# Malfoy/Brisk

Hardware: AMD Instinct MI355X
Metric: distinct k-mers indexed/sec (k=63,m=21) (higher is better)
Workload: dtype u64; 1 GPU; 1x MI355X: 50M synthetic 150 bp reads per GPU, k=63 m=21 b=14, uint8 counts, 15x coverage; reads_per_gpu=50000000, total_reads=50000000, part_bits=24, genome_len=500000000, parallelism=single GPU

## Files before the change

### brisk_amd/csrc/brisk_scan.hip

```cpp
__global__ void __launch_bounds__(256) k_pack_ascii(const uint8_t* __restrict__ bases, u64 n_bases, u32* __restrict__ packed, u64 n_words) {
    const u64 w = (u64)blockIdx.x * blockDim.x + threadIdx.x;
    if (w >= n_words) return;
    const u64 base = w * 16;
    u32 v = 0;
    if (base + 16 <= n_bases && ((uintptr_t)(bases + base) & 15) == 0) {
        const uint4 q = *reinterpret_cast<const uint4*>(bases + base);
        const u32 ws[4] = {q.x, q.y, q.z, q.w};
#pragma unroll
        for (int i = 0; i < 4; i++) {
#pragma unroll
            for (int j = 0; j < 4; j++) v = (v << 2) | ((ws[i] >> (8 * j + 1)) & 3u);
        }
    } else {
        for (int i = 0; i < 16; i++) {
            const u64 p = base + i;
            const u32 c = p < n_bases ? ((bases[p] >> 1) & 3u) : 0u;
            v = (v << 2) | c;
        }
    }
    packed[w] = v;
}

__device__ __forceinline__ u64 sm_mix(u64 z) {
    z = (z ^ (z >> 30)) * 0xBF58476D1CE4E5B9ull;
// ... 117 lines not shown
                s.rev = c != fwd;
            } else if (d == s.pos) {
                if (canon < 0) {
                    const u64 hi = K > 32 ? load_nts(packed, q, K - 32) : 0;
                    canon = canonized_as_executed(mk128(low, hi), K) ? 1 : 0;
                }
                if (!canon) {
                    s.pos = d;
                    s.mini = c;
                    s.rev = false;
                }
            }
        }
    }
    return s;
}

template <bool CLS>
__device__ __forceinline__ u32 superkmer_pieces(const BriskParams& P, u32 n, u32 idx_end) {
    return (CLS ? P.cls_bits : 0u) ? cls_of(P, idx_end) - cls_of(P, idx_end - (n - 1)) + 1 : 1u;
}

__device__ __forceinline__ W4 x_shr(W4 a, u32 s) { return w4_shr(a, s); }
__device__ __forceinline__ W4 x_shl(W4 a, u32 s) { return w4_shl(a, s); }
__device__ __forceinline__ W4 x_and(W4 a, W4 b) { return w4_and(a, b); }
__device__ __forceinline__ W4 x_andn(W4 a, W4 b) { return w4_andn(a, b); }
__device__ __forceinline__ W4 x_or(W4 a, W4 b) { return w4_or(a, b); }
__device__ __forceinline__ W4 x_xor(W4 a, W4 b) { return W4{a.w0 ^ b.w0, a.w1 ^ b.w1, a.w2 ^ b.w2, a.w3 ^ b.w3}; }
__device__ __forceinline__ W4 x_rc(W4 a, u32 len) { return w4_rc(a, len); }
__device__ __forceinline__ u64 x_w0(W4 a) { return a.w0; }
__device__ __forceinline__ u64 x_word(W4 a, u32 i) { return i == 0 ? a.w0 : i == 1 ? a.w1 : i == 2 ? a.w2 : a.w3; }
__device__ __forceinline__ u128x x_shr(u128x a, u32 s) { return shr128(a, s); }
__device__ __forceinline__ u128x x_shl(u128x a, u32 s) { return shl128(a, s); }
__device__ __forceinline__ u128x x_and(u128x a, u128x b) { return and128(a, b); }
__device__ __forceinline__ u128x x_andn(u128x a, u128x b) { return andn128(a, b); }
__device__ __forceinline__ u128x x_or(u128x a, u128x b) { return or128(a, b); }
__device__ __forceinline__ u128x x_xor(u128x a, u128x b) { return u128x{a.lo ^ b.lo, a.hi ^ b.hi}; }
__device__ __forceinline__ u128x x_rc(u128x a, u32 len) {
    const u64 c = 0xaaaaaaaaaaaaaaaaull;
    return shr128(u128x{rev_nts64(a.hi ^ c), rev_nts64(a.lo ^ c)}, 128 - 2 * len);
}
__device__ __forceinline__ u64 x_w0(u128x a) { return a.lo; }
__device__ __forceinline__ u64 x_word(u128x a, u32 i) { return i == 0 ? a.lo : i == 1 ? a.hi : 0ull; }
template <class T> __device__ __forceinline__ T x_mask(u32 bits);
template <> __device__ __forceinline__ W4 x_mask<W4>(u32 bits) { return w4_mask(bits); }
template <> __device__ __forceinline__ u128x x_mask<u128x>(u32 bits) { return mask128(bits); }
template <class T> __device__ __forceinline__ T x_from64(u64 v);
template <> __device__ __forceinline__ W4 x_from64<W4>(u64 v) { return W4{v, 0, 0, 0}; }
template <> __device__ __forceinline__ u128x x_from64<u128x>(u64 v) { return u128x{v, 0}; }
template <class T> __device__ __forceinline__ T x_load(const u32* __restrict__ packed, u64 q, u32 len);
template <> __device__ __forceinline__ W4 x_load<W4>(const u32* __restrict__ packed, u64 q, u32 len) { return load_span(packed, q, len); }
template <> __device__ __forceinline__ u128x x_load<u128x>(const u32* __restrict__ packed, u64 q, u32 len) {
    const u32 c = len >= 32 ? 32 : len;
    u128x r{load_nts(packed, q + len - c, c), 0};
    if (len > 32) r.hi = load_nts(packed, q, len - 32);
    return r;
}

template <bool CLS, class T, bool POS = false>
__device__ __forceinline__ void emit_record_wide(const BriskParams& P, const u32* __restrict__ packed, u64 q0, u32 p0, u32 n, bool rev,
                                                 u32 idx_end, const ScanOut& out, u32 tag, u64 ret, unsigned long long slot) {
    const u32 L = P.k + n - 1;
    T S = x_load<T>(packed, q0 + p0, L);
    if (rev) S = x_rc(S, L);
    const u64 mm = x_w0(x_shr(S, 2 * idx_end)) & P.m_mask;
    const u64 h = mix2m(mm, P.m_mask);
    const u32 rbase = routing_base(P, h);
    S = x_xor(S, x_shl(x_from64<T>(mm ^ h), 2 * idx_end));
    const u32 cut = idx_end + P.suff_reduc;
    const T lowm = x_mask<T>(2 * cut);
    const T C = x_or(x_andn(x_shr(S, 2 * P.b), lowm), x_and(S, lowm));
    const u32 idx_first = idx_end - (n - 1);

    for (u32 j0 = 0; j0 < n;) {
        u32 j1 = n, bucket = rbase;
        if ((CLS ? P.cls_bits : 0u)) {
            const u32 c = cls_of(P, idx_first + j0);
            if (c + 1 < (1u << (CLS ? P.cls_bits : 0u))) j1 = min(n, (c + 1) * P.cls_width - idx_first);
            bucket = (rbase << (CLS ? P.cls_bits : 0u)) | c;
        }
        const u32 np = j1 - j0;
        T Cp = C;
        if (np != n) Cp = x_and(x_shr(C, 2 * (n - j1)), x_mask<T>(2 * (P.kb + np - 1)));
        u64* r;
        if (out.bins) {
            const u32 part = bucket >> P.shift;
#ifdef SCAN_ATTR_NOATOMIC
            const u32 rank = (part * 7u + (threadIdx.x & 63)) % out.bin_cap;
#else
            const u32 rank = (u32)atomicAdd(&out.hist[part], 1ull | ((unsigned long long)np << 32));
#endif
            if (rank < out.bin_cap) {
                r = out.bins + ((u64)part * out.bin_cap + rank) * P.stride;
                if (POS) {
                    const u64 ti = (u64)part * out.bin_cap + rank;
                    out.tag[ti] = (u32)ti;
                    out.ret[ti] = ret;
                } else if (out.tag) out.tag[(u64)part * out.bin_cap + rank] = tag;
            } else {
                const u32 reg = part & (OVF_REGIONS - 1);
                const u32 at = atomicAdd(&out.ovf_cnt[reg], 1u);
                if (at >= out.ovf_region_cap) {
                    *out.overflow = 1;
                    return;
                }
                const u64 o = (u64)reg * out.ovf_region_cap + at;
                r = out.ovf + o * P.stride;
                if (POS) {
                    const u64 ti = ((u64)out.bin_cap << P.part_bits) + o;
                    out.tag[ti] = (u32)ti;
                    out.ret[ti] = ret;
                } else if (out.tag) out.tag[((u64)out.bin_cap << P.part_bits) + o] = tag;
            }
        } else {
            r = out.rec + slot * P.stride;
        }
#ifdef SCAN_ATTR_NOSTORE
        if ((x_word(Cp, 0) ^ x_word(Cp, 1)) == 0x123456789abcdefull)
#endif
        {
            r[0] = x_word(Cp, 0);
            if (P.nw > 1) r[1] = x_word(Cp, 1);
            if (P.nw > 2) r[2] = x_word(Cp, 2);
            if (P.nw > 3) r[3] = x_word(Cp, 3);
            r[P.nw] = rec_header(bucket, np, idx_first + j0 + P.suff_reduc);
        }
        if (!out.bins) {
            if (out.tag) out.tag[slot] = tag;
            if (out.ret) out.ret[slot] = ret;
            if (out.hist) atomicAdd(&out.hist[bucket >> P.shift], 1ull | ((unsigned long long)np << 32));
        }
        slot++;
        j0 = j1;
    }
}
#ifndef EMIT_SMALL
#define EMIT_SMALL 1
#endif
template <bool CLS, bool POS = false>
__device__ void emit_record_at(const BriskParams& P, const u32* __restrict__ packed, u64 q0, u32 p0, u32 n, bool rev,
                               u32 idx_end, const ScanOut& out, u32 tag, u64 ret, unsigned long long slot) {
    if (!out.bins && slot + superkmer_pieces<CLS>(P, n, idx_end) > out.cap) {
        *out.overflow = 1;
        return;
    }
    if (EMIT_SMALL && 2 * P.k - P.m <= 64) emit_record_wide<CLS, u128x, POS>(P, packed, q0, p0, n, rev, idx_end, out, tag, ret, slot);
    else emit_record_wide<CLS, W4, POS>(P, packed, q0, p0, n, rev, idx_end, out, tag, ret, slot);
}
__device__ void emit_record(const BriskParams& P, const u32* __restrict__ packed, u64 q0, u32 p0, u32 n, bool rev,
                            u32 idx_end, const ScanOut& out, u32 tag, u64 ret = 0) {
    emit_record_at<true>(P, packed, q0, p0, n, rev, idx_end, out, tag, ret, atomicAdd(out.n_rec, (unsigned long long)superkmer_pieces<true>(P, n, idx_end)));
}

__global__ void __launch_bounds__(SCAN_BLOCK) k_scan(BriskParams P, const u32* __restrict__ packed, const u64* __restrict__ starts,
                                                     u64 n_reads, const double* __restrict__ g_coef, ScanOut out, int query_mode) {
    __shared__ double s_coef[128];
    for (u32 i = threadIdx.x; i < 4 * P.m; i += blockDim.x) s_coef[i] = g_coef[i];
    __syncthreads();
    const u64 r = (u64)blockIdx.x * blockDim.x + threadIdx.x;
    if (r >= n_reads) return;
    const u64 q0 = starts[r];
    const u64 len = starts[r + 1] - q0;
    const u32 k = P.k, m = P.m, w = P.w;
    if (len < k) return;
    const u64 M = P.m_mask;

    u64 cf = 0, cr = 0;
    for (u32 i = 0; i < m; i++) {
        const u32 c = nt_at(packed, q0 + k - m - 1 + i);
        cf = ((cf << 2) + c) & (M >> 2);
        cr = (cr >> 2) + ((u64)(c ^ 2u) << (2 * m - 2));
    }
    MiniState st = rescan_minimizer(packed, q0, k - 1, m, M, s_coef);
    u64 mini_hash = order_key(st.mini, m, M, s_coef);
    u32 mini_pos = st.pos;
    bool reversed = st.rev;
    u64 mini = st.mini;

    const u32 nk = (u32)(len - k + 1);
    u32 n = 0, p0 = 0, first_idx = 0, last_idx = 0, n_emitted = 0;
    for (u32 p = 0; p < nk; p++) {
        const u32 c = nt_at(packed, q0 + k - 1 + p);
        cf = ((cf << 2) + c) & M;
        cr = (cr >> 2) + ((u64)(c ^ 2u) << (2 * m - 2));
        mini_pos++;
        const u64 cand = cf < cr ? cf : cr;
        const u64 h = order_key(cand, m, M, s_coef);
        bool closed = false;
        const bool old_rev = reversed;
        u64 ret = 0;
        if (mini_pos > w) {
            closed = true;
            ret = mini;
            st = rescan_minimizer(packed, q0 + p, k, m, M, s_coef);
            mini = st.mini;
            mini_pos = st.pos;
            reversed = st.rev;
            mini_hash = order_key(mini, m, M, s_coef);
        } else if (h < mini_hash) {
            closed = true;
            ret = mini;
            mini_hash = h;
            mini_pos = 0;
            mini = cand;
            reversed = cand == cr;
        }
        const u32 idx = reversed ? w - mini_pos : mini_pos;
        if (closed && p > 0) {
            if (query_mode && n_emitted > 0 && ret == 0) return;
            emit_record(P, packed, q0, p0, n, old_rev, old_rev ? first_idx : last_idx, out, out.ret ? p0 : (u32)r, ret);
            n_emitted++;
            n = 0;
        }
        if (n == 0) {
            p0 = p;
            first_idx = idx;
        }
        last_idx = idx;
        n++;
    }
    if (n > 0) {
        if (query_mode && n_emitted > 0 && mini == 0) return;
        emit_record(P, packed, q0, p0, n, reversed, reversed ? first_idx : last_idx, out, out.ret ? p0 : (u32)r, mini);
    }
}

__device__ __forceinline__ unsigned long long lanes_below(u32 lane) { return (1ull << lane) - 1; }

#ifndef CLS_W
#define CLS_W 5
#endif
__host__ __device__ constexpr u32 cls_nch(u32 m) { return (m + CLS_W - 1) / CLS_W; }
__host__ __device__ constexpr u32 cls_width(u32 m, u32 c) {
    return m / cls_nch(m) + (c < m % cls_nch(m) ? 1u : 0u);
}
__host__ __device__ constexpr u32 cls_off(u32 m, u32 c) {
    u32 o = 0;
    for (u32 j = 0; j < c; j++) o += cls_width(m, j);
    return o;
}
__host__ __device__ constexpr u32 cls_base(u32 m, u32 c) {
    u32 b = 0;
    for (u32 j = 0; j < c; j++) b += 1u << (2 * cls_width(m, j));
    return b;
}
#define CLS_MAX_CHUNKS 8

struct ScanCfg {
    u32 nlow;
    u32 nlow1;
    u32 nch;
    u32 qcap;
    u32 n_tab;
    u32 chunk[CLS_MAX_CHUNKS];
};

#define CLS_HI 21
#define CLS_LO 12
#define CLS_BIAS 0x80000000u
__host__ __device__ constexpr u32 scan_fixed_tabs(int MM) { return MM > 0 ? 128 + cls_base((u32)MM, cls_nch((u32)MM)) : 0u; }
template <int NCH, int MM>
__device__ __forceinline__ u64 cls_sums(u64 x, const ScanCfg& cfg, const u64* tabs) {
    u64 acc;
    if (MM > 0) {
        constexpr u32 mm = MM > 0 ? (u32)MM : 1u;
        const char* tb = (const char*)tabs;
        const u32 xl = (u32)x, xh = (u32)(x >> 32);
        acc = *(const u64*)(tb + ((xl << 3) & (((1u << (2 * cls_width(mm, 0))) - 1) << 3)));
#pragma unroll
        for (u32 c = 1; c < cls_nch(mm); c++) {
            const u32 lo = 2 * cls_off(mm, c), wd = 2 * cls_width(mm, c), mk = ((1u << wd) - 1) << 3;
            u32 bo;
            if (lo + wd <= 32) bo = xl >> (lo - 3);
            else if (lo >= 35) bo = xh >> (lo - 35);
            else if (lo >= 32) bo = xh << (35 - lo);
            else bo = (u32)(x >> (lo - 3));
            acc += *(const u64*)(tb + 8 * cls_base(mm, c) + (bo & mk));
        }
    } else if (NCH > 0) {
        acc = tabs[(u32)x & ((1u << ((cfg.chunk[0] >> 6) & 15)) - 1)];
#pragma unroll
        for (int c = 1; c < NCH; c++) {
            const u32 d = cfg.chunk[c];
            acc += tabs[(d >> 10) + ((u32)(x >> (d & 63)) & ((1u << ((d >> 6) & 15)) - 1))];
        }
    } else {
        acc = tabs[(u32)x & ((1u << ((cfg.chunk[0] >> 6) & 15)) - 1)];
        for (u32 c = 1; c < cfg.nch; c++) {
            const u32 d = cfg.chunk[c];
            acc += tabs[(d >> 10) + ((u32)(x >> (d & 63)) & ((1u << ((d >> 6) & 15)) - 1))];
        }
    }
    return acc;
}
template <int NCH, int MM>
__device__ __forceinline__ u32 decy_class_guarded(u64 x, const ScanCfg& cfg, const u64* tabs, bool& guard) {
    const u64 acc = cls_sums<NCH, MM>(x, cfg, tabs);
    const u32 a = (u32)acc, b = (u32)(acc >> 32);
    const u32 da = ((a > CLS_BIAS ? a : CLS_BIAS) - (a < CLS_BIAS ? a : CLS_BIAS)) + (0u - (CLS_LO + 1));
    const u32 db = ((b > CLS_BIAS ? b : CLS_BIAS) - (b < CLS_BIAS ? b : CLS_BIAS)) + (0u - (CLS_LO + 1));
    guard = guard | ((da < db ? da : db) <= (u32)(CLS_HI - CLS_LO - 2));
    const bool c0 = a >= CLS_BIAS + CLS_HI && b <= CLS_BIAS + CLS_LO, c1 = a <= CLS_BIAS - CLS_HI && b >= CLS_BIAS - CLS_LO;
#ifdef CLS_FORCE_GUARD
    guard = true;
#endif
    return c0 ? 0u : c1 ? 1u : 2u;
// ... 169 lines not shown
    const u32 slot = tags[i];
    if (i < n_spec_end && (status[slot] & CHUNK_RERUN)) return;
    const u64 r = ret[i], q = r & 0x7fffffffffffffffull;
    const VRead v = vreads[slot];
    if ((r >> 63) && q > starts[v.read]) atomicMin(&brk[v.first], (unsigned long long)q);
}
__global__ void __launch_bounds__(256) k_query_filter(BriskParams P, const u64* __restrict__ rec, const u64* __restrict__ ret, const u32* __restrict__ tags, u64 first,
                                                      u64 n_spec_end, u64 n_rec, const VRead* __restrict__ vreads, const u32* __restrict__ status,
                                                      const unsigned long long* __restrict__ brk, u64* __restrict__ out, u32* __restrict__ tag_out,
                                                      unsigned long long* __restrict__ n_out) {
    const u64 i = first + (u64)blockIdx.x * blockDim.x + threadIdx.x;
    if (i >= n_rec) return;
    const u32 slot = tags[i];
    if (i < n_spec_end && (status[slot] & CHUNK_RERUN)) return;
    const VRead v = vreads[slot];
    if ((ret[i] & 0x7fffffffffffffffull) >= brk[v.first]) return;
    const unsigned long long o = atomicAdd(n_out, 1ull);
    for (u32 j = 0; j < P.stride; j++) out[o * P.stride + j] = rec[i * P.stride + j];
    tag_out[o] = v.read;
}
__global__ void __launch_bounds__(256) k_filter_records(BriskParams P, const u64* __restrict__ rec, const u32* __restrict__ tags, u64 first, u64 n_rec,
                                                        const u32* __restrict__ status, u64* __restrict__ out, unsigned long long* __restrict__ n_out) {
    const u64 i = first + (u64)blockIdx.x * blockDim.x + threadIdx.x;
    if (i >= n_rec) return;
    if (status[tags[i]] & CHUNK_RERUN) return;
    const unsigned long long slot = atomicAdd(n_out, 1ull);
    for (u32 j = 0; j < P.stride; j++) out[slot * P.stride + j] = rec[i * P.stride + j];
}

#define SLOT_ITEMS 16
__device__ __forceinline__ u64 read_slots(const u64* __restrict__ starts, u64 r, u32 k) {
    const u64 len = starts[r + 1] - starts[r];
    return len >= k ? len - k + 1 : 0;
}
__global__ void __launch_bounds__(256) k_slot_block(const u64* __restrict__ starts, u64 n_reads, u32 k, u64* __restrict__ block_sums) {
    __shared__ u64 s[4];
    const u64 base = (u64)blockIdx.x * 256 * SLOT_ITEMS;
    u64 acc = 0;
    for (int i = 0; i < SLOT_ITEMS; i++) {
        const u64 r = base + (u64)i * 256 + threadIdx.x;
        if (r < n_reads) acc += read_slots(starts, r, k);
    }
    for (int o = 32; o > 0; o >>= 1) acc += __shfl_down(acc, o, 64);
    if ((threadIdx.x & 63) == 0) s[threadIdx.x >> 6] = acc;
    __syncthreads();
    if (threadIdx.x == 0) block_sums[blockIdx.x] = s[0] + s[1] + s[2] + s[3];
}
__global__ void __launch_bounds__(1024) k_slot_top(u64* __restrict__ block_sums, u32 nb) {
    __shared__ u64 s_wave[16];
    __shared__ u64 s_carry;
    if (threadIdx.x == 0) s_carry = 0;
    __syncthreads();
    for (u32 base = 0; base < nb; base += 1024) {
        const u32 i = base + threadIdx.x;
        const u64 v = i < nb ? block_sums[i] : 0;
        u64 x = v;
        for (int o = 1; o < 64; o <<= 1) {
            const u64 y = __shfl_up(x, o, 64);
            if ((int)(threadIdx.x & 63) >= o) x += y;
        }
        if ((threadIdx.x & 63) == 63) s_wave[threadIdx.x >> 6] = x;
        __syncthreads();
        u64 woff = 0;
        for (u32 j = 0; j < (threadIdx.x >> 6); j++) woff += s_wave[j];
        const u64 carry = s_carry;
        if (i < nb) block_sums[i] = carry + woff + x - v;
        __syncthreads();
        if (threadIdx.x == 1023) s_carry = carry + woff + x;
        __syncthreads();
    }
    if (threadIdx.x == 0) block_sums[nb] = s_carry;
}
__global__ void __launch_bounds__(256) k_slot_apply(const u64* __restrict__ starts, u64 n_reads, u32 k, const u64* __restrict__ block_sums,
                                                    u64* __restrict__ slot_base) {
    __shared__ u64 s_wave[4];
    const u64 base = (u64)blockIdx.x * 256 * SLOT_ITEMS + (u64)threadIdx.x * SLOT_ITEMS;
    u64 tsum = 0;
    for (int i = 0; i < SLOT_ITEMS; i++)
        if (base + i < n_reads) tsum += read_slots(starts, base + i, k);
    u64 x = tsum;
    for (int o = 1; o < 64; o <<= 1) {
        const u64 y = __shfl_up(x, o, 64);
        if ((int)(threadIdx.x & 63) >= o) x += y;
    }
    if ((threadIdx.x & 63) == 63) s_wave[threadIdx.x >> 6] = x;
    __syncthreads();
    u64 woff = 0;
    for (u32 j = 0; j < (threadIdx.x >> 6); j++) woff += s_wave[j];
    u64 run = block_sums[blockIdx.x] + woff + x - tsum;
    for (int i = 0; i < SLOT_ITEMS; i++) {
        const u64 r = base + i;
        if (r >= n_reads) break;
        slot_base[r] = run - starts[r];
        run += read_slots(starts, r, k);
    }
}
__global__ void __launch_bounds__(256) k_chunk_slot_base(const VRead* __restrict__ vreads, u32 n_chunks, const u64* __restrict__ slot_base, u64* __restrict__ out) {
    const u32 i = blockIdx.x * blockDim.x + threadIdx.x;
    if (i < n_chunks) out[i] = slot_base[vreads[i].read];
}
__global__ void __launch_bounds__(256) k_pos_filter(BriskParams P, const u64* __restrict__ rec, const u64* __restrict__ anchor, const u32* __restrict__ tags, u64 first,
                                                    u64 n_spec_end, u64 n_rec, const u32* __restrict__ status, u64* __restrict__ out, u64* __restrict__ anchor_out,
                                                    unsigned long long* __restrict__ n_out) {
    const u64 i = first + (u64)blockIdx.x * blockDim.x + threadIdx.x;
    if (i >= n_rec) return;
    if (i < n_spec_end && (status[tags[i]] & CHUNK_RERUN)) return;
    const unsigned long long o = atomicAdd(n_out, 1ull);
    for (u32 j = 0; j < P.stride; j++) out[o * P.stride + j] = rec[i * P.stride + j];
    anchor_out[o] = anchor[i];
}

__device__ __forceinline__ void resolve_ties(u32 first, u32 last, bool rev_first, bool rev_last, u32 Km, bool canon_if_needed_known, bool canon,
                                             u32* pos, bool* rev, bool* need_canon) {
    *need_canon = false;
    *pos = first;
    *rev = rev_first;
    if (last != first) {
        const u32 dT = Km - last;
        if (dT < first) {
            *pos = dT;
            *rev = rev_last;
        } else if (dT == first) {
            if (!canon_if_needed_known) *need_canon = true;
            else if (!canon) *rev = false;
        }
    }
}

__device__ __forceinline__ u64 pos_anchor(const BriskParams& P, u64 slot_base, u64 q, u32 n, bool rev, u32 idx_end) {
    const u64 g = rev ? q + idx_end : q + P.w - idx_end + n - 1;
    return (slot_base + g) | (rev ? 1ull << 63 : 0ull);
}

template <bool CLS, bool POS = false>
__device__ __forceinline__ void emit_queued(const BriskParams& P, const u32* __restrict__ packed, const ScanOut& out, u64 ent, const u64* s_q0, const u32* s_tag,
                                            unsigned long long slot, const u64* slot_base) {
    const u32 mi = (u32)(ent >> 32), src = (mi >> 18) & 63u;
    const u64 q_start = s_q0[src] + (u32)ent;
    const u64 ret = POS ? pos_anchor(P, slot_base[s_tag[src]], q_start, mi & 0xff, (mi >> 16) & 1, (mi >> 8) & 0xff) : q_start | ((u64)((mi >> 17) & 1) << 63);
    emit_record_at<CLS, POS>(P, packed, q_start, 0, mi & 0xff, (mi >> 16) & 1, (mi >> 8) & 0xff, out, s_tag[src], ret, slot);
}

template <bool CLS>
__device__ __forceinline__ u32 queue_records(const BriskParams& P, const u64* q_ent, u32 qcount) {
    if (!(CLS ? P.cls_bits : 0u)) return qcount;
    u32 mine = 0;
    for (u32 e = threadIdx.x & 63; e < qcount; e += 64) {
        const u32 mi = (u32)(q_ent[e] >> 32);
        mine += superkmer_pieces<CLS>(P, mi & 0xff, (mi >> 8) & 0xff);
    }
    for (int o = 32; o > 0; o >>= 1) mine += __shfl_xor(mine, o, 64);
    return mine;
}
template <bool CLS, bool POS = false>
__device__ __forceinline__ void emit_queue(const BriskParams& P, const u32* __restrict__ packed, const ScanOut& out, const u64* q_ent, const u64* s_q0, const u32* s_tag,
                                           u32 qcount, unsigned long long base, const u64* slot_base = nullptr) {
    const u32 lane = threadIdx.x & 63;
    if (!(CLS ? P.cls_bits : 0u)) {
        for (u32 e = lane; e < qcount; e += 64) emit_queued<CLS, POS>(P, packed, out, q_ent[e], s_q0, s_tag, base + e, slot_base);
        return;
    }
    for (u32 e0 = 0; e0 < qcount; e0 += 64) {
        const u32 e = e0 + lane;
        u64 ent = 0;
        u32 np = 0;
        if (e < qcount) {
            ent = q_ent[e];
            const u32 mi = (u32)(ent >> 32);
            np = superkmer_pieces<CLS>(P, mi & 0xff, (mi >> 8) & 0xff);
        }
        u32 incl = np;
        for (int o = 1; o < 64; o <<= 1) {
            const u32 y = __shfl_up(incl, o, 64);
            if ((int)lane >= o) incl += y;
        }
        if (e < qcount) emit_queued<CLS, POS>(P, packed, out, ent, s_q0, s_tag, base + incl - np, slot_base);
        base += (u32)__shfl(incl, 63, 64);
    }
}

template <bool CLS, bool POS = false>
__device__ __forceinline__ void scan_final_flush(const BriskParams& P, const u32* __restrict__ packed, const ScanOut& out, const u64* q_ent, const u64* s_q0,
                                                 const u32* s_tag, u32 qcount, u32* s_wcnt, unsigned long long* s_wbase, const u64* slot_base = nullptr) {
    const u32 lane = threadIdx.x & 63, wid = threadIdx.x >> 6, nw = blockDim.x >> 6;
    const u32 n_mine = queue_records<CLS>(P, q_ent, qcount);
    if (out.bins) {
        if (lane == 0 && n_mine) atomicAdd(out.n_rec, (unsigned long long)n_mine);
        emit_queue<CLS, POS>(P, packed, out, q_ent, s_q0, s_tag, qcount, 0, slot_base);
        return;
    }
    if (lane == 0) s_wcnt[wid] = n_mine;
    __syncthreads();
    if (threadIdx.x == 0) {
        u32 total = 0;
        for (u32 i = 0; i < nw; i++) total += s_wcnt[i];
        *s_wbase = total ? atomicAdd(out.n_rec, (unsigned long long)total) : 0ull;
    }
    __syncthreads();
    unsigned long long base = *s_wbase;
    for (u32 i = 0; i < wid; i++) base += s_wcnt[i];
    emit_queue<CLS, POS>(P, packed, out, q_ent, s_q0, s_tag, qcount, base, slot_base);
}

__device__ __forceinline__ u32 row_min_u32(u32 x) {
#define ROW_MIN_STEP(CTRL)                                                                      \
    {                                                                                           \
        const u32 y_ = (u32)__builtin_amdgcn_update_dpp((int)x, (int)x, CTRL, 0xf, 0xf, false); \
        x = y_ < x ? y_ : x;                                                                    \
    }
    ROW_MIN_STEP(0x128)
    ROW_MIN_STEP(0x124)
    ROW_MIN_STEP(0x122)
    ROW_MIN_STEP(0x121)
#undef ROW_MIN_STEP
    return x;
}

struct MinQueue {
    u64 k0, k1, k2;
    u32 meta;
};
#define MQ_EMPTY (~0ull)
#define MQ_TRUNC (1u << 30)
__device__ __forceinline__ void mq_reset(MinQueue& q, u64 key, u32 birth, bool rv, bool trunc) {
    q.k0 = key;
    q.k1 = q.k2 = MQ_EMPTY;
    q.meta = (birth & 0xffu) | (rv ? 1u << 24 : 0u) | (trunc ? MQ_TRUNC : 0u);
}
__device__ __forceinline__ void mq_push(MinQueue& q, u64 h, u32 step, bool rv) {
    const bool l0 = q.k0 < h, l1 = q.k1 < h, l2 = q.k2 < h;
    const bool e0 = q.k0 == h, e1 = q.k1 == h, e2 = q.k2 == h;
    const u32 cnt = (q.k0 != MQ_EMPTY ? 1u : 0u) + (q.k1 != MQ_EMPTY ? 1u : 0u) + (q.k2 != MQ_EMPTY ? 1u : 0u);
    const u32 keep = (l0 ? 1u : 0u) + (l1 ? 1u : 0u) + (l2 ? 1u : 0u);
    if (e0 | e1 | e2) {
        const u32 j = e0 ? 0u : e1 ? 1u : 2u;
        if (j < 1) q.k1 = MQ_EMPTY;
        if (j < 2) q.k2 = MQ_EMPTY;
        q.meta |= (1u << (27 + j)) | MQ_TRUNC;
        return;
    }
    const bool store = keep < 3 && (!(q.meta & MQ_TRUNC) || keep < cnt);
    if (!store) {
        q.meta |= MQ_TRUNC;
        return;
    }
    const u32 sh = 8 * keep;
    q.meta = (q.meta & ~((0xffu << sh) | (1u << (24 + keep)) | (1u << (27 + keep)) | MQ_TRUNC)) | ((step & 0xffu) << sh) | (rv ? 1u << (24 + keep) : 0u);
    if (keep == 0) q.k0 = h;
    if (keep <= 1) q.k1 = keep == 1 ? h : MQ_EMPTY;
    if (keep <= 2) q.k2 = keep == 2 ? h : MQ_EMPTY;
}
__device__ __forceinline__ void mq_pop_front(MinQueue& q) {
    q.k0 = q.k1;
    q.k1 = q.k2;
    q.k2 = MQ_EMPTY;
    q.meta = ((q.meta >> 8) & 0xffffu) | (((q.meta >> 25) & 3u) << 24) | (((q.meta >> 28) & 3u) << 27) | (q.meta & MQ_TRUNC);
}

#ifdef BRISK_PHASE_PROF
__device__ unsigned long long g_scan_cnt[8];
#define SCNT(i, v) scan_cnt[i] += (v);
#else
#define SCNT(i, v)
#endif

#ifndef SCAN_WAVES_PER_EU
#define SCAN_WAVES_PER_EU 6
#endif
__host__ __device__ constexpr int scan_waves_per_eu(int KK, int MM) { return KK && MM >= 12 ? SCAN_WAVES_PER_EU : 4; }
template <int NCH, int MODE, int KK, int MM>
__global__ void __launch_bounds__(1024) __attribute__((amdgpu_waves_per_eu(scan_waves_per_eu(KK, MM), 8))) k_scan2(BriskParams P, ScanCfg cfg, const u32* __restrict__ packed, const u64* __restrict__ starts,
                                                u64 n_reads, const double* __restrict__ g_tabs, ScanOut out, ChunkCtl cc) {
    constexpr bool VR = MODE == 2 || MODE == 4, query_mode = MODE == 1, POS = MODE >= 3;
    constexpr bool CLS = MM < 12;
    extern __shared__ double smem_dyn[];
    const u32 tid = threadIdx.x, lane = tid & 63, wid = tid >> 6;
    const u32 n_tab = MM ? 128 + cls_base(MM ? MM : 1, cls_nch(MM ? MM : 1)) : cfg.n_tab;
    double* smem_d = smem_dyn;
    double* smem_q = smem_dyn + n_tab;
    if constexpr (scan_fixed_tabs(MM) > 0) {
        __shared__ double s_fix[scan_fixed_tabs(MM)];
        smem_d = s_fix;
        smem_q = smem_dyn;
    }
    const double* s_coef = smem_d;
    const u64* s_tabs = (const u64*)(smem_d + 128);
    for (u32 i = tid; i < n_tab; i += blockDim.x) smem_d[i] = g_tabs[i];
    unsigned long long* s_wbase = (unsigned long long*)smem_q;
    u32* s_wcnt = (u32*)(s_wbase + 1);
    u64* q_ent = (u64*)(smem_q + 9) + (size_t)wid * (cfg.qcap + 96);
    u64* s_q0 = q_ent + cfg.qcap;
    u32* s_tag = (u32*)(s_q0 + 64);

    if (KK) {
        P.k = KK;
        P.w = KK - MM;
    }
    if (MM) {
        P.m = MM;
        P.m_mask = (1ull << (2 * MM)) - 1;
    }
    const u32 k = KK ? (u32)KK : P.k, m = MM ? (u32)MM : P.m, w = k - m;
    const u64 M = MM ? ((1ull << (2 * MM)) - 1) : P.m_mask;
    const u32 ksh = 2 * m > 30 ? 2 * m - 30 : 0;
    const u32 nlow = k < 32 ? k : 32, nlow1 = k - 1 < 32 ? k - 1 : 32;
    const u64 r = (u64)blockIdx.x * blockDim.x + tid;
    u64 q0 = 0, len = 0;
    u32 emit_from = 0, emit_until = 0xffffffffu, tagval = (u32)r, vslot = 0;
    bool seq_first = true, seq_last = true, seeded = false;
    if (r < n_reads) {
        if (VR) {
            const VRead v = cc.vreads[r];
            q0 = v.q0;
            len = v.len;
            emit_from = v.emit_from;
            emit_until = v.emit_until;
            tagval = vslot = v.slot;
            seq_first = v.flags & 1u;
            seq_last = v.flags & 2u;
            seeded = v.flags & 4u;
        } else {
            q0 = starts[r];
            len = starts[r + 1] - q0;
            if (cc.long_limit && len >= k && len - k + 1 > cc.long_limit) len = 0;
        }
    }
    s_q0[lane] = q0;
    s_tag[lane] = tagval;
    __syncthreads();
    const bool live = len >= k;
    u32 nk = live ? (u32)(len - k + 1) : 0;
    u32 max_nk = nk;
    for (int o = 32; o > 0; o >>= 1) {
        const u32 y = __shfl_xor(max_nk, o, 64);
        max_nk = y > max_nk ? y : max_nk;
    }
    if (max_nk == 0) {
        scan_final_flush<CLS, POS>(P, packed, out, q_ent, s_q0, s_tag, 0, s_wcnt, s_wbase, cc.slot_base);
        return;
    }
    const u64 KEY0 = order_key_fast<NCH, MM>(0, m, M, cfg, s_tabs, s_coef);
    const u64 KEY0s = read_lane_u64(KEY0, 0);

    u64 cr = 0, low64 = 0;
    if (live) low64 = load_nts(packed, q0 + (k - 1) - nlow1, nlow1);
    cr = rc64(low64 & M, m);

    u64 mini_hash;
    u32 mini_pos;
    bool reversed;
#ifndef SCAN_MINQUEUE
#define SCAN_MINQUEUE 1
#endif
#ifndef PROLOGUE_UNROLL
#define PROLOGUE_UNROLL 2
#endif
#define BRISK_PRAGMA_(x) _Pragma(#x)
#define BRISK_PRAGMA(x) BRISK_PRAGMA_(x)
    const bool mq_on = SCAN_MINQUEUE && (KK ? (KK <= 32) : (k <= 32));
    MinQueue mq{MQ_EMPTY, MQ_EMPTY, MQ_EMPTY, 0u};
    {
        const u32 Km = k - 1 - m;
        const u32 nwin = Km + 1 < nlow1 ? Km + 1 : nlow1;
        struct WinMin {
            u64 best;
            u32 first, last, flags;
        };
        auto pass = [&](auto exact_tag) -> WinMin {
            constexpr bool EXACT = decltype(exact_tag)::value;
            u64 best = ~0ull;
            u32 first = 0, last = 0, rf = 0, rl = 0;
            bool guard = false;
            u64 fw = low64 & M, rw = cr, above = low64 >> (2 * m);
            if (mq_on) mq = MinQueue{MQ_EMPTY, MQ_EMPTY, MQ_EMPTY, 0u};
#ifdef SCAN_ATTR_NOPROLOGUE
            for (u32 ii = 0; ii < 1; ii++) {
#else
            BRISK_PRAGMA(unroll PROLOGUE_UNROLL)
            for (u32 ii = 0; ii < nwin; ii++) {
#endif
                const u32 i = mq_on ? Km - ii : ii;
                u64 fwd, rcv;
                if (mq_on) {
                    fwd = (low64 >> (2 * i)) & M;
                    rcv = rc64(fwd, m);
                } else {
                    fwd = fw;
                    rcv = rw;
                    const u32 t = (u32)above & 3u;
                    above >>= 2;
                    fw = (fw >> 2) | ((u64)t << (2 * m - 2));
                    rw = ((rw << 2) & M) | (t ^ 2u);
                }
                const bool rv = rcv < fwd;
                const u64 x = rv ? rcv : fwd;
                u64 key;
                if (EXACT) key = order_key(x, m, M, s_coef);
                else {
#ifdef SCAN_ATTR_NOCLASS
                    key = order_key_fast<NCH, MM>(x, m, M, cfg, s_tabs, s_coef);
#else
                    key = ((u64)decy_class_guarded<NCH, MM>(x, cfg, s_tabs, guard) << 62) + mix2m(x, M);
#endif
                }
                const bool lt = key < best, eq = key == best;
                best = lt ? key : best;
                if (mq_on) {
                    first = lt || eq ? i : first;
                    rf = lt || eq ? (u32)rv : rf;
                    last = lt ? i : last;
                    rl = lt ? (u32)rv : rl;
                } else {
                    first = lt ? i : first;
                    rf = lt ? (u32)rv : rf;
                    last = lt || eq ? i : last;
                    rl = lt || eq ? (u32)rv : rl;
                }
                if (mq_on) mq_push(mq, key, 0u - 1u - i, rv);
            }
            return WinMin{best, first, last, rf | (rl << 1) | (guard ? 4u : 0u)};
        };
#ifdef SCAN_ATTR_PROLOGUE_TWICE
        if (__ballot(pass(std::false_type{}).flags & 4u) == 0x123456789ull) return;
        __builtin_amdgcn_s_barrier();
#endif
        WinMin wm = pass(std::false_type{});
        if (__ballot(wm.flags & 4u)) wm = pass(std::true_type{});
        u64 best = wm.best;
        u32 first = wm.first, last = wm.last;
        bool rf = wm.flags & 1u, rl = wm.flags & 2u;
        if (Km >= nwin) {
            if (KEY0 < best) {
                best = KEY0;
                first = nwin;
                last = Km;
                rf = rl = false;
            } else if (KEY0 == best) {
                last = Km;
                rl = false;
            }
        }
        u32 pos;
        bool rev, need_canon;
        resolve_ties(first, last, rf, rl, Km, false, false, &pos, &rev, &need_canon);
        if (need_canon && live) {
            const u64 hi = k - 1 > 32 ? load_nts(packed, q0, k - 1 - 32) : 0;
            if (!canonized_as_executed(mk128(low64, hi), k - 1)) rev = false;
        }
        mini_hash = best;
        mini_pos = pos;
        reversed = rev;
        if (mq_on && last != first) mq_reset(mq, best, 0u - 1u - pos, rev, true);
    }
    if (seeded) {
        const ChunkState st = cc.truth[vslot];
        mini_hash = st.hash;
        mini_pos = st.pos_rev & 0x7fffffffu;
        reversed = st.pos_rev >> 31;
        if (mq_on) mq_reset(mq, mini_hash, 0u - 1u - mini_pos, reversed, true);
    }
    bool foreign = seeded;

    u32 qcount = 0;
    u32 p0 = 0, n_emitted = 0;
    bool dead = false;
    u64 buf = 0;
    const u32 Km = k - m;
    const u32 lane_bits = lane << 18;
#ifdef BRISK_PHASE_PROF
    unsigned long long scan_cnt[8] = {0, 0, 0, 0, 0, 0, 0, 0};
#endif
    for (u32 p = 0; p < max_nk; p++) {
        SCNT(0, 1)
        const bool act = p < nk && !dead;
        if (VR && live) {
            if (p == emit_from && !seq_first && !seeded) cc.spec[vslot] = ChunkState{mini_hash, mini_pos | ((reversed ? 1u : 0u) << 31), 1u};
            if (p == emit_until) cc.truth[vslot + 1] = ChunkState{mini_hash, mini_pos | ((reversed ? 1u : 0u) << 31), 1u};
        }
        if ((p & 31) == 0 && p < nk) {
            const u32 left = (u32)(len - (k - 1 + p));
            const u32 cnt = left < 32 ? left : 32;
            buf = load_nts(packed, q0 + k - 1 + p, cnt) << (64 - 2 * cnt);
        }
        const u32 c = (u32)(buf >> 62);
        buf <<= 2;
        cr = (cr >> 2) + ((u64)(c ^ 2u) << (2 * m - 2));
        low64 = (low64 << 2) | c;
        const u64 cf = low64 & M;
        const bool revf = cr < cf;
        const u64 h = order_key_fast<NCH, MM>(revf ? cr : cf, m, M, cfg, s_tabs, s_coef);
        mini_pos += act ? 1u : 0u;
        if (mq_on) mq_push(mq, h, p, revf);
        const bool expired = act && mini_pos > w;
        const bool newmin = act && !expired && h < mini_hash;
        const bool closed = expired || newmin;
        bool push = closed && p > 0 && !foreign && p0 >= emit_from && p0 < emit_until;
        if (closed) foreign = false;
        if (query_mode && push && n_emitted > 0 && mini_hash == KEY0) {
            push = false;
            dead = true;
        }
        {
            const unsigned long long bal = __ballot(push);
            if (push) {
                const u32 n = p - p0;
                const u32 idx_end = reversed ? w + n - mini_pos : mini_pos - 1;
                const u32 hi = n | (idx_end << 8) | ((reversed ? 1u : 0u) << 16) | ((mini_hash == KEY0 ? 1u : 0u) << 17) | lane_bits;
                q_ent[qcount + (u32)__popcll(bal & lanes_below(lane))] = ((u64)hi << 32) | p0;
                if (query_mode) n_emitted++;
            }
            qcount += (u32)__popcll(bal);
            SCNT(4, (u32)__popcll(bal))
        }
        bool served = false;
        if (mq_on && expired && mq.k0 != MQ_EMPTY && ((p - mq.meta) & 0xffu) == mini_pos) {
            mq_pop_front(mq);
            if (mq.k0 != MQ_EMPTY && !(mq.meta & (1u << 27))) {
                mini_hash = mq.k0;
                mini_pos = (p - mq.meta) & 0xffu;
                reversed = (mq.meta >> 24) & 1u;
                served = true;
            }
        }
        unsigned long long need = __ballot(expired && !dead && !served);
        SCNT(6, (u32)__popcll(__ballot(served)))
        SCNT(1, (u32)__popcll(need))
#ifdef SCAN_ATTR_NORESCAN
        if (expired) {
            mini_pos = 0;
            mini_hash = h;
        }
        need = 0;
#endif
        while (need) {
            const int LA = __ffsll((long long)need) - 1;
            need &= need - 1;
            const bool two = need != 0;
            SCNT(2, 1)
            SCNT(3, two ? 1 : 0)
            int LB = LA;
            if (two) {
                LB = __ffsll((long long)need) - 1;
                need &= need - 1;
            }
            const u64 lowA = read_lane_u64(low64, LA), lowB = read_lane_u64(low64, LB);
            const u32 wl = lane & 31;
            const u64 lowL = lane < 32 ? lowA : lowB;
            const u64 fwd = (lowL >> (2 * wl)) & M;
            const u64 rcv = rc64(fwd, m);
            const bool rv = rcv < fwd;
            u64 key = order_key_fast<NCH, MM>(rv ? rcv : fwd, m, M, cfg, s_tabs, s_coef);
            u32 k32 = ((u32)(key >> 62) << 30) | (u32)((key & M) >> ksh);
            if (wl > Km || wl >= nlow) {
                key = ~0ull;
                k32 = ~0u;
            }
            const u32 rm = row_min_u32(k32);
            const u32 r0 = (u32)__builtin_amdgcn_readlane((int)rm, 0), r1 = (u32)__builtin_amdgcn_readlane((int)rm, 16);
            const u32 r2 = (u32)__builtin_amdgcn_readlane((int)rm, 32), r3 = (u32)__builtin_amdgcn_readlane((int)rm, 48);
            const u32 mA = r0 < r1 ? r0 : r1, mB = r2 < r3 ? r2 : r3;
            unsigned long long tie = __ballot(k32 == (lane < 32 ? mA : mB));
            const unsigned long long rvb = __ballot(rv);
            const bool unique = __popc((u32)tie) == 1 && (!two || __popc((u32)(tie >> 32)) == 1);
            u64 hm = key;
            if (!unique) {
                for (int o = 16; o > 0; o >>= 1) {
                    const u64 y = __shfl_xor(hm, o, 64);
                    hm = y < hm ? y : hm;
                }
                tie = __ballot(key == hm);
            }
#ifdef SCAN_ATTR_RS_NOEPI
            if ((int)lane == LA || (two && (int)lane == LB)) {
                mini_hash = key;
                mini_pos = (u32)tie & 31u;
                reversed = rv;
            }
            if (false)
#endif
            for (int half = 0; half < (two ? 2 : 1); half++) {
                const int L = half ? LB : LA;
                const u32 t = (u32)(tie >> (32 * half)), rb = (u32)(rvb >> (32 * half));
                u32 first = (u32)__ffs((int)t) - 1, last = 31u - (u32)__clz((int)t);
                u64 hmin = unique ? read_lane_u64(key, 32 * half + (int)first) : read_lane_u64(hm, 32 * half);
                bool rf = (rb >> first) & 1, rl = (rb >> last) & 1;
                if (Km >= 32) {
                    if (KEY0s < hmin) {
                        hmin = KEY0s;
                        first = 32;
                        last = Km;
                        rf = rl = false;
                    } else if (KEY0s == hmin) {
                        last = Km;
                        rl = false;
                    }
                }
                u32 pos;
                bool rev, need_canon;
                resolve_ties(first, last, rf, rl, Km, false, false, &pos, &rev, &need_canon);
                if (need_canon) {
                    const u64 lowX = half ? lowB : lowA;
                    const u64 qL = read_lane_u64(q0, L) + p;
                    const u64 hi = k > 32 ? load_nts(packed, qL, k - 32) : 0;
                    const u64 lo = k >= 32 ? lowX : (lowX & ((1ull << (2 * k)) - 1));
                    if (!canonized_as_executed(mk128(lo, hi), k)) rev = false;
                }
                if ((int)lane == L) {
                    mini_hash = hmin;
                    mini_pos = pos;
                    reversed = rev;
                    if (mq_on) mq_reset(mq, hmin, p - pos, rev, pos != 0);
                }
            }
        }
        if (newmin) {
            mini_hash = h;
            mini_pos = 0;
            reversed = revf;
            if (mq_on) mq_reset(mq, h, p, revf, false);
        }
        if (closed && (p > 0 || seeded)) p0 = p;
        if (qcount + 64 > cfg.qcap) {
#ifndef SCAN_ATTR_NOEMIT
            const u32 n_out = queue_records<CLS>(P, q_ent, qcount);
            unsigned long long base = 0;
            if (out.bins) {
                if (lane == 0) atomicAdd(out.n_rec, (unsigned long long)n_out);
            } else {
                if (lane == 0) base = atomicAdd(out.n_rec, (unsigned long long)n_out);
                base = read_lane_u64(base, 0);
            }
            emit_queue<CLS, POS>(P, packed, out, q_ent, s_q0, s_tag, qcount, base, cc.slot_base);
#endif
            qcount = 0;
        }
    }
    {
        bool push = live && !dead && nk > p0 && seq_last && !foreign && p0 >= emit_from && p0 < emit_until;
        if (push && query_mode && n_emitted > 0 && mini_hash == KEY0) push = false;
        const unsigned long long bal = __ballot(push);
        if (push) {
            const u32 n = nk - p0;
            const u32 idx_end = reversed ? w + n - 1 - mini_pos : mini_pos;
            const u32 hi = n | (idx_end << 8) | ((reversed ? 1u : 0u) << 16) | ((mini_hash == KEY0 ? 1u : 0u) << 17) | lane_bits;
            q_ent[qcount + (u32)__popcll(bal & lanes_below(lane))] = ((u64)hi << 32) | p0;
        }
        qcount += (u32)__popcll(bal);
    }
#ifdef BRISK_PHASE_PROF
    if (lane == 0)
        for (int i = 0; i < 8; i++) atomicAdd(&g_scan_cnt[i], scan_cnt[i]);
#endif
#ifdef SCAN_ATTR_NOEMIT
    qcount = 0;
#endif
    scan_final_flush<CLS, POS>(P, packed, out, q_ent, s_q0, s_tag, qcount, s_wcnt, s_wbase, cc.slot_base);
}
```

Measured before the change: 30.74 billion k-mers/s.

## Add specialized anchored super-k-mer emission path for k=63, m=21

Adds a compile-time specialized record emitter for k=63/m=21 that loads a fixed seven-word frame ending at the super-k-mer's last nucleotide. It builds the record with alignbit shifts, masks, minimizer hashing and suffix reduction in registers instead of the generic wide-integer emit path. A block-wide upper word bound is computed so queue entries near buffer edges fall back to the generic path. It also makes wave ids scalar via readfirstlane and changes the DPP row-min to use -1 as the bound-control fill value. This adds an extra reduction and sync per block, plus a correctness risk in the hand-derived bit masks.

```diff
diff --git a/brisk_amd/csrc/brisk_scan.hip b/brisk_amd/csrc/brisk_scan.hip
--- a/brisk_amd/csrc/brisk_scan.hip
+++ b/brisk_amd/csrc/brisk_scan.hip
@@ -293,6 +293,127 @@
     emit_record_at<true>(P, packed, q0, p0, n, rev, idx_end, out, tag, ret, atomicAdd(out.n_rec, (unsigned long long)superkmer_pieces<true>(P, n, idx_end)));
 }
 
+#define AF_K 63
+#define AF_M 21
+#define AF_W (AF_K - AF_M)
+#define AF_DW 7
+#define AF_MIN (2 * AF_W)
+struct Frame7 {
+    u32 d0, d1, d2, d3, d4, d5, d6;
+};
+__device__ __forceinline__ u32 af_align(u32 hi, u32 lo, u32 s) { return __builtin_amdgcn_alignbit(hi, lo, s); }
+__device__ __forceinline__ u32 rc_nts32(u32 x) {
+    const u32 r = __brev(x ^ 0xaaaaaaaau);
+    return ((r >> 1) & 0x55555555u) | ((r & 0x55555555u) << 1);
+}
+__device__ __forceinline__ u32 af_low_ones(int h) {
+    const u32 c = (u32)min(max(h, 0), 16);
+    return (~0u >> c) >> c;
+}
+__device__ __forceinline__ u64 af_last_nt(u64 q, u32 n, bool rev, u32 idx_end) {
+    return rev ? q + idx_end + (16 * AF_DW - 1 - AF_W) : q + (AF_K + n - 1) + (AF_W - 1) - idx_end;
+}
+__device__ __forceinline__ Frame7 anchored_record(const BriskParams& P, const u32* __restrict__ packed, u64 e, u32 n, bool rev, u32 idx_end, u32* rbase) {
+    const u32* p = packed + (e >> 4);
+    const u32 sh = 30 - 2 * ((u32)e & 15);
+    const u32 l0 = p[0], l1 = p[-1], l2 = p[-2], l3 = p[-3], l4 = p[-4], l5 = p[-5], l6 = p[-6], l7 = p[-7];
+    Frame7 f{af_align(l1, l0, sh), af_align(l2, l1, sh), af_align(l3, l2, sh), af_align(l4, l3, sh), af_align(l5, l4, sh), af_align(l6, l5, sh), af_align(l7, l6, sh)};
+    if (rev) f = Frame7{rc_nts32(f.d6), rc_nts32(f.d5), rc_nts32(f.d4), rc_nts32(f.d3), rc_nts32(f.d2), rc_nts32(f.d1), rc_nts32(f.d0)};
+    const u32 idx_first = idx_end - (n - 1);
+    const int pre = (int)(AF_W - idx_first);
+    f.d3 &= pre ? ~0u : 0x3fffffffu;
+    f.d4 &= af_low_ones(17 - pre);
+    f.d5 &= af_low_ones(33 - pre);
+    f.d6 &= (1u << (u32)max(2 * pre - 66, 0)) - 1;
+    u64 mid = ((u64)f.d3 << 32) | f.d2;
+    const u64 mm = (mid >> (AF_MIN - 64)) & P.m_mask;
+    const u64 h = mix2m(mm, P.m_mask);
+    *rbase = routing_base(P, h);
+    mid ^= (mm ^ h) << (AF_MIN - 64);
+    f.d2 = (u32)mid;
+    f.d3 = (u32)(mid >> 32);
+    {
+        u32 geo = P.b | (P.suff_reduc << 8);
+        asm volatile("" : "+s"(geo));
+        const u32 c0 = AF_MIN + 2 * (geo >> 8), s = 2 * (geo & 0xff), bs = s & 31;
+        const bool ws = s >= 32;
+        const u32 a2 = ws ? f.d3 : f.d2, a3 = ws ? f.d4 : f.d3, a4 = ws ? f.d5 : f.d4, a5 = ws ? f.d6 : f.d5, a6 = ws ? 0u : f.d6;
+        const u32 r2 = af_align(a3, a2, bs), r3 = af_align(a4, a3, bs), r4 = af_align(a5, a4, bs), r5 = af_align(a6, a5, bs), r6 = a6 >> bs;
+        const u32 lm2 = c0 >= 96 ? ~0u : (1u << (c0 - 64)) - 1, lm3 = c0 <= 96 ? 0u : (1u << (c0 - 96)) - 1;
+        f.d2 = (f.d2 & lm2) | (r2 & ~lm2);
+        f.d3 = (f.d3 & lm3) | (r3 & ~lm3);
+        f.d4 = r4;
+        f.d5 = r5;
+        f.d6 = r6;
+    }
+    {
+        const u32 s = AF_MIN - 2 * idx_end, ws = s >> 5, bs = s & 31;
+        const u32 t0 = ws == 0 ? f.d0 : ws == 1 ? f.d1 : f.d2, t1 = ws == 0 ? f.d1 : ws == 1 ? f.d2 : f.d3, t2 = ws == 0 ? f.d2 : ws == 1 ? f.d3 : f.d4;
+        const u32 t3 = ws == 0 ? f.d3 : ws == 1 ? f.d4 : f.d5, t4 = ws == 0 ? f.d4 : ws == 1 ? f.d5 : f.d6, t5 = ws == 0 ? f.d5 : ws == 1 ? f.d6 : 0u;
+        const u32 t6 = ws == 0 ? f.d6 : 0u;
+        f = Frame7{af_align(t1, t0, bs), af_align(t2, t1, bs), af_align(t3, t2, bs), af_align(t4, t3, bs), af_align(t5, t4, bs), af_align(t6, t5, bs), t6 >> bs};
+    }
+    return f;
+}
+template <bool POS>
+__device__ __forceinline__ void emit_record_anchored(const BriskParams& P, const u32* __restrict__ packed, u64 e, u32 n, bool rev, u32 idx_end, const ScanOut& out,
+                                                     u32 tag, u64 ret, unsigned long long slot) {
+    if (!out.bins && slot + 1 > out.cap) {
+        *out.overflow = 1;
+        return;
+    }
+    u32 bucket;
+    const Frame7 f = anchored_record(P, packed, e, n, rev, idx_end, &bucket);
+    u64* r;
+    if (out.bins) {
+        const u32 part = bucket >> P.shift;
+#ifdef SCAN_ATTR_NOATOMIC
+        const u32 rank = (part * 7u + (threadIdx.x & 63)) % out.bin_cap;
+#else
+        const u32 rank = (u32)atomicAdd(&out.hist[part], 1ull | ((unsigned long long)n << 32));
+#endif
+        if (rank < out.bin_cap) {
+            r = out.bins + ((u64)part * out.bin_cap + rank) * P.stride;
+            if (POS) {
+                const u64 ti = (u64)part * out.bin_cap + rank;
+                out.tag[ti] = (u32)ti;
+                out.ret[ti] = ret;
+            } else if (out.tag) out.tag[(u64)part * out.bin_cap + rank] = tag;
+        } else {
+            const u32 reg = part & (OVF_REGIONS - 1);
+            const u32 at = atomicAdd(&out.ovf_cnt[reg], 1u);
+            if (at >= out.ovf_region_cap) {
+                *out.overflow = 1;
+                return;
+            }
+            const u64 o = (u64)reg * out.ovf_region_cap + at;
+            r = out.ovf + o * P.stride;
+            if (POS) {
+                const u64 ti = ((u64)out.bin_cap << P.part_bits) + o;
+                out.tag[ti] = (u32)ti;
+                out.ret[ti] = ret;
+            } else if (out.tag) out.tag[((u64)out.bin_cap << P.part_bits) + o] = tag;
+        }
+    } else {
+        r = out.rec + slot * P.stride;
+    }
+#ifdef SCAN_ATTR_NOSTORE
+    if ((f.d0 ^ f.d2) == 0x12345678u && f.d1 == 0x9abcdefu)
+#endif
+    {
+        r[0] = ((u64)f.d1 << 32) | f.d0;
+        if (P.nw > 1) r[1] = ((u64)f.d3 << 32) | f.d2;
+        if (P.nw > 2) r[2] = ((u64)f.d5 << 32) | f.d4;
+        if (P.nw > 3) r[3] = f.d6;
+        r[P.nw] = rec_header(bucket, n, idx_end - (n - 1) + P.suff_reduc);
+    }
+    if (!out.bins) {
+        if (out.tag) out.tag[slot] = tag;
+        if (out.ret) out.ret[slot] = ret;
+        if (out.hist) atomicAdd(&out.hist[bucket >> P.shift], 1ull | ((unsigned long long)n << 32));
+    }
+}
+
 __global__ void __launch_bounds__(SCAN_BLOCK) k_scan(BriskParams P, const u32* __restrict__ packed, const u64* __restrict__ starts,
                                                      u64 n_reads, const double* __restrict__ g_coef, ScanOut out, int query_mode) {
     __shared__ double s_coef[128];
@@ -768,10 +889,29 @@
     for (int o = 32; o > 0; o >>= 1) mine += __shfl_xor(mine, o, 64);
     return mine;
 }
-template <bool CLS, bool POS = false>
+template <bool CLS, bool POS = false, bool ANCH = false>
 __device__ __forceinline__ void emit_queue(const BriskParams& P, const u32* __restrict__ packed, const ScanOut& out, const u64* q_ent, const u64* s_q0, const u32* s_tag,
-                                           u32 qcount, unsigned long long base, const u64* slot_base = nullptr) {
+                                           u32 qcount, unsigned long long base, const u64* slot_base = nullptr, u32 hi_word = 0) {
     const u32 lane = threadIdx.x & 63;
+    if constexpr (ANCH && !CLS) {
+        u32 e0 = 0;
+        for (; e0 < qcount; e0 += 64) {
+            const u32 e = e0 + lane;
+            const bool act = e < qcount;
+            const u64 ent = act ? q_ent[e] : 0;
+            const u32 mi = (u32)(ent >> 32), src = (mi >> 18) & 63u, n = mi & 0xff, idx_end = (mi >> 8) & 0xff;
+            const bool rev = (mi >> 16) & 1;
+            const u64 q_start = s_q0[src] + (u32)ent;
+            const u64 last = af_last_nt(q_start, n, rev, idx_end), wl = last >> 4;
+            if (__ballot(act && (wl < AF_DW || wl > hi_word))) break;
+            if (act) {
+                const u64 ret = POS ? pos_anchor(P, slot_base[s_tag[src]], q_start, n, rev, idx_end) : q_start | ((u64)((mi >> 17) & 1) << 63);
+                emit_record_anchored<POS>(P, packed, last, n, rev, idx_end, out, s_tag[src], ret, base + e);
+            }
+        }
+        for (u32 e = e0 + lane; e < qcount; e += 64) emit_queued<CLS, POS>(P, packed, out, q_ent[e], s_q0, s_tag, base + e, slot_base);
+        return;
+    }
     if (!(CLS ? P.cls_bits : 0u)) {
         for (u32 e = lane; e < qcount; e += 64) emit_queued<CLS, POS>(P, packed, out, q_ent[e], s_q0, s_tag, base + e, slot_base);
         return;
@@ -795,14 +935,15 @@
     }
 }
 
-template <bool CLS, bool POS = false>
+template <bool CLS, bool POS = false, bool ANCH = false>
 __device__ __forceinline__ void scan_final_flush(const BriskParams& P, const u32* __restrict__ packed, const ScanOut& out, const u64* q_ent, const u64* s_q0,
-                                                 const u32* s_tag, u32 qcount, u32* s_wcnt, unsigned long long* s_wbase, const u64* slot_base = nullptr) {
-    const u32 lane = threadIdx.x & 63, wid = threadIdx.x >> 6, nw = blockDim.x >> 6;
+                                                 const u32* s_tag, u32 qcount, u32* s_wcnt, unsigned long long* s_wbase, const u64* slot_base = nullptr, u32 hi_word = 0) {
+    const u32 lane = threadIdx.x & 63, nw = blockDim.x >> 6;
+    const u32 wid = ANCH ? (u32)__builtin_amdgcn_readfirstlane(threadIdx.x >> 6) : threadIdx.x >> 6;
     const u32 n_mine = queue_records<CLS>(P, q_ent, qcount);
     if (out.bins) {
         if (lane == 0 && n_mine) atomicAdd(out.n_rec, (unsigned long long)n_mine);
-        emit_queue<CLS, POS>(P, packed, out, q_ent, s_q0, s_tag, qcount, 0, slot_base);
+        emit_queue<CLS, POS, ANCH>(P, packed, out, q_ent, s_q0, s_tag, qcount, 0, slot_base, hi_word);
         return;
     }
     if (lane == 0) s_wcnt[wid] = n_mine;
@@ -815,14 +956,17 @@
     __syncthreads();
     unsigned long long base = *s_wbase;
     for (u32 i = 0; i < wid; i++) base += s_wcnt[i];
-    emit_queue<CLS, POS>(P, packed, out, q_ent, s_q0, s_tag, qcount, base, slot_base);
-}
-
+    emit_queue<CLS, POS, ANCH>(P, packed, out, q_ent, s_q0, s_tag, qcount, base, slot_base, hi_word);
+}
+
+#ifndef ROW_MIN_FOLD
+#define ROW_MIN_FOLD 1
+#endif
 __device__ __forceinline__ u32 row_min_u32(u32 x) {
-#define ROW_MIN_STEP(CTRL)                                                                      \
-    {                                                                                           \
-        const u32 y_ = (u32)__builtin_amdgcn_update_dpp((int)x, (int)x, CTRL, 0xf, 0xf, false); \
-        x = y_ < x ? y_ : x;                                                                    \
+#define ROW_MIN_STEP(CTRL)                                                                                               \
+    {                                                                                                                    \
+        const u32 y_ = (u32)__builtin_amdgcn_update_dpp(ROW_MIN_FOLD ? -1 : (int)x, (int)x, CTRL, 0xf, 0xf, false);      \
+        x = y_ < x ? y_ : x;                                                                                             \
     }
     ROW_MIN_STEP(0x128)
     ROW_MIN_STEP(0x124)
@@ -889,8 +1033,10 @@
                                                 u64 n_reads, const double* __restrict__ g_tabs, ScanOut out, ChunkCtl cc) {
     constexpr bool VR = MODE == 2 || MODE == 4, query_mode = MODE == 1, POS = MODE >= 3;
     constexpr bool CLS = MM < 12;
+    constexpr bool ANCH = KK == AF_K && MM == AF_M;
     extern __shared__ double smem_dyn[];
-    const u32 tid = threadIdx.x, lane = tid & 63, wid = tid >> 6;
+    const u32 tid = threadIdx.x, lane = tid & 63;
+    const u32 wid = ANCH ? (u32)__builtin_amdgcn_readfirstlane(tid >> 6) : tid >> 6;
     const u32 n_tab = MM ? 128 + cls_base(MM ? MM : 1, cls_nch(MM ? MM : 1)) : cfg.n_tab;
     double* smem_d = smem_dyn;
     double* smem_q = smem_dyn + n_tab;
@@ -943,7 +1089,19 @@
     }
     s_q0[lane] = q0;
     s_tag[lane] = tagval;
+    u32 hi_word = 0;
+    if constexpr (ANCH) {
+        const u64 hw = len >= k ? ((q0 + len - 1) >> 4) + 2 : 0;
+        hi_word = hw > 0xffffffffull ? 0xffffffffu : (u32)hw;
+        for (int o = 32; o > 0; o >>= 1) hi_word = max(hi_word, (u32)__shfl_xor(hi_word, o, 64));
+        if (lane == 0) s_wcnt[wid] = hi_word;
+    }
     __syncthreads();
+    if constexpr (ANCH) {
+        for (u32 i = 0; i < (blockDim.x >> 6); i++) hi_word = max(hi_word, s_wcnt[i]);
+        hi_word = __builtin_amdgcn_readfirstlane(hi_word);
+        __syncthreads();
+    }
     const bool live = len >= k;
     u32 nk = live ? (u32)(len - k + 1) : 0;
     u32 max_nk = nk;
@@ -952,7 +1110,7 @@
         max_nk = y > max_nk ? y : max_nk;
     }
     if (max_nk == 0) {
-        scan_final_flush<CLS, POS>(P, packed, out, q_ent, s_q0, s_tag, 0, s_wcnt, s_wbase, cc.slot_base);
+        scan_final_flush<CLS, POS, ANCH>(P, packed, out, q_ent, s_q0, s_tag, 0, s_wcnt, s_wbase, cc.slot_base, hi_word);
         return;
     }
     const u64 KEY0 = order_key_fast<NCH, MM>(0, m, M, cfg, s_tabs, s_coef);
@@ -1246,7 +1404,7 @@
                 if (lane == 0) base = atomicAdd(out.n_rec, (unsigned long long)n_out);
                 base = read_lane_u64(base, 0);
             }
-            emit_queue<CLS, POS>(P, packed, out, q_ent, s_q0, s_tag, qcount, base, cc.slot_base);
+            emit_queue<CLS, POS, ANCH>(P, packed, out, q_ent, s_q0, s_tag, qcount, base, cc.slot_base, hi_word);
 #endif
             qcount = 0;
         }
@@ -1270,5 +1428,5 @@
 #ifdef SCAN_ATTR_NOEMIT
     qcount = 0;
 #endif
-    scan_final_flush<CLS, POS>(P, packed, out, q_ent, s_q0, s_tag, qcount, s_wcnt, s_wbase, cc.slot_base);
-}
+    scan_final_flush<CLS, POS, ANCH>(P, packed, out, q_ent, s_q0, s_tag, qcount, s_wcnt, s_wbase, cc.slot_base, hi_word);
+}
```

After: 31.23 billion k-mers/s (median of 6 runs). 1.02x the previous value.
